# Lynx-MR/orbslam3lib

Measured on AMD Instinct MI355X. Metric: Mfeatures/s extract + Mmatches/s BFMatch, 640x480 stereo 8-level pyr, 1/2/4/8 GPU, higher is better.
Workload: dtype u8; 1 GPU; C2 640x480 stereo, 8 levels x1.2, 2000 feat/frame, FAST 20/7, + per-pair 2000x2000 Hamming kNN2 (left->right, all rows); parallelism=frames sharded across 1 GPU(s), replicas

## Files before the change

### orbslam3lib_amd/csrc/orb_knn2.hip

```cpp
#include <hip/hip_runtime.h>
#include <stdint.h>

#include <algorithm>
#include <type_traits>

#include "orb_kernels.h"

namespace orbgpu {

__device__ inline uint32_t med3_u32(uint32_t a, uint32_t b, uint32_t c) {
    return max(min(a, b), min(max(a, b), c));
}

__device__ inline void knn2_store(uint32_t k1, uint32_t k2, int qi, int32_t* i1, int32_t* d1,
                                  int32_t* i2, int32_t* d2) {
    i1[qi] = k1 == 0xFFFFFFFFu ? -1 : (int32_t)(k1 & 0xFFFF);
    d1[qi] = k1 == 0xFFFFFFFFu ? 0x7fffffff : (int32_t)(k1 >> 16);
    i2[qi] = k2 == 0xFFFFFFFFu ? -1 : (int32_t)(k2 & 0xFFFF);
    d2[qi] = k2 == 0xFFFFFFFFu ? 0x7fffffff : (int32_t)(k2 >> 16);
}

typedef int knn_v8i __attribute__((ext_vector_type(8)));
typedef float knn_v16f __attribute__((ext_vector_type(16)));
constexpr int kKnnWaves = 8;
constexpr int kKnnThreads = 64 * kKnnWaves;
constexpr int kKnnQ = 32 * kKnnWaves;
static_assert(kKnnQ == kKnnQueries, "orb_kernels.h kKnnQueries (grid and arrival counters)");
constexpr int kKnnSeg = 4096;
constexpr int kKnnPitch4 = 144;
__device__ inline uint32_t knn_nib_of(uint32_t ws) {
    uint32_t r;
    asm("v_and_or_b32 %0, %1, %2, %3" : "=v"(r) : "v"(ws), "v"(0x88888888u), "v"(0x22222222u));
    return r;
}
__device__ inline knn_v8i knn4_expand(uint32_t w) {
    knn_v8i v;
    v[0] = (int)knn_nib_of(w << 3);
    v[1] = (int)knn_nib_of(w << 2);
    v[2] = (int)knn_nib_of(w << 1);
    v[3] = (int)knn_nib_of(w);
    v[4] = v[5] = v[6] = v[7] = 0;
    return v;
}
__device__ inline float knn_med3_f32(float a, float b, float c) {
    float r;
    asm("v_med3_f32 %0, %1, %2, %3" : "=v"(r) : "v"(a), "v"(b), "v"(c));
    return r;
}
__device__ inline float knn_max3_f32(float a, float b, float c) {
    float r;
    asm("v_max3_f32 %0, %1, %2, %3" : "=v"(r) : "v"(a), "v"(b), "v"(c));
    return r;
}
__device__ __attribute__((always_inline)) inline void knn2_fp4_block(
    const uint8_t* q, int nq, const uint8_t* t, int nt, int qb, int ts, int te, int32_t* i1, int32_t* d1,
    int32_t* i2, int32_t* d2, uint2* part, uint8_t* lds) {
    const int tid = threadIdx.x, lane = tid & 63, wave = tid >> 6;
    const int r = lane & 31, h = lane >> 5;
    const int qi = qb * kKnnQ + wave * 32 + r;
    knn_v8i qf[4];
    {
        const uint4* qp = reinterpret_cast<const uint4*>(q + (long long)min(qi, max(nq - 1, 0)) * 32);
        const uint4 qa = qp[0], qc = qp[1];
        qf[0] = knn4_expand(h ? qa.y : qa.x);
        qf[1] = knn4_expand(h ? qa.w : qa.z);
        qf[2] = knn4_expand(h ? qc.y : qc.x);
        qf[3] = knn4_expand(h ? qc.w : qc.z);
    }
    uint32_t g1 = 0xFFFFFFFFu, g2 = 0xFFFFFFFFu;
    const int er = tid >> 3, ed = tid & 7;
    const bool expander = tid < 256;
    auto load_packed = [&](int tile) __attribute__((always_inline)) {
        const int row = min(tile * 32 + er, nt - 1);
        return expander ? *reinterpret_cast<const uint32_t*>(t + (long long)row * 32 + 4 * ed) : 0u;
    };
    auto tile_lds = [&](int u) __attribute__((always_inline)) { return lds + ((u - ts) & 1) * (32 * kKnnPitch4); };
    auto store_expanded = [&](int u, uint32_t w) __attribute__((always_inline)) {
        if (expander) {
            const knn_v8i v = knn4_expand(w);
            *reinterpret_cast<uint4*>(tile_lds(u) + er * kKnnPitch4 + 16 * ed) = make_uint4(v[0], v[1], v[2], v[3]);
        }
    };
    uint32_t pk0 = 0, pk1 = 0;
    if (te > ts) {
        store_expanded(ts, load_packed(ts));
        pk1 = load_packed(ts + 1);
    }
    auto rowc = [](int g) { return (g & 3) + 8 * (g >> 2); };
    knn_v16f C0;
#pragma unroll
    for (int g = 0; g < 16; ++g) C0[g] = (float)(4095 - 4 * h - rowc(g));
    const float kNone = -1073741824.0f;
    for (int seg0 = (ts * 32 / kKnnSeg) * kKnnSeg; seg0 < te * 32; seg0 += kKnnSeg) {
        const int tile0 = max(seg0 >> 5, ts), tile1 = min(te, (seg0 + kKnnSeg) >> 5);
        float ka1 = kNone, ka2 = kNone, kb1 = kNone, kb2 = kNone;
        auto select = [&](const knn_v16f& v, bool shift) __attribute__((always_inline)) {
            if (shift) {
                ka1 += 32.f;
                ka2 += 32.f;
                kb1 += 32.f;
                kb2 += 32.f;
            }
#pragma unroll
            for (int g = 0; g < 16; g += 4) {
                const float x0 = v[g], y0 = v[g + 1], x1 = v[g + 2], y1 = v[g + 3];
                ka2 = fmaxf(ka2, knn_med3_f32(ka1, x0, y0));
                ka1 = knn_max3_f32(ka1, x0, y0);
                kb2 = fmaxf(kb2, knn_med3_f32(kb1, x1, y1));
                kb1 = knn_max3_f32(kb1, x1, y1);
            }
        };
        auto body = [&](int ti, auto par, knn_v16f& acc, const knn_v16f& prev) __attribute__((always_inline)) {
            constexpr int PAR = decltype(par)::value;
            uint32_t& pk_use = PAR ? pk0 : pk1;
            uint32_t& pk_load = PAR ? pk1 : pk0;
            __syncthreads();
            pk_load = load_packed(ti + 2);
            const uint8_t* ab = tile_lds(ti) + r * kKnnPitch4 + 16 * h;
#pragma unroll
            for (int s = 0; s < 4; ++s) {
                const uint4 a4 = *reinterpret_cast<const uint4*>(ab + 32 * s);
                const knn_v8i a = {(int)a4.x, (int)a4.y, (int)a4.z, (int)a4.w, 0, 0, 0, 0};
                acc = __builtin_amdgcn_mfma_scale_f32_32x32x64_f8f6f4(a, qf[s], s ? acc : C0, 4, 4, 0, 133, 0, 133);
            }
            if (ti > tile0) select(prev, ti - 1 > tile0);
            if (ti + 1 < te) store_expanded(ti + 1, pk_use);
            if (ti * 32 + 32 > nt) {
#pragma unroll
                for (int g = 0; g < 16; ++g)
                    if (ti * 32 + rowc(g) + 4 * h >= nt) acc[g] = kNone;
            }
        };
        using P0 = std::integral_constant<int, 0>;
        using P1 = std::integral_constant<int, 1>;
        knn_v16f acc0, acc1;
        int ti = tile0;
        for (; ti + 1 < tile1; ti += 2) {
            body(ti, P0{}, acc0, acc1);
            body(ti + 1, P1{}, acc1, acc0);
        }
        if (ti < tile1) {
            body(ti, P0{}, acc0, acc1);
            select(acc0, ti > tile0);
        } else if (tile1 > tile0) {
            select(acc1, tile1 - 1 > tile0);
        }
        const int unbias = 32 * (tile1 - 1 - tile0);
        const int k1 = (int)fmaxf(ka1, kb1) - unbias;
        const int k2 = (int)fmaxf(fminf(ka1, kb1), fmaxf(ka2, kb2)) - unbias;
        auto fold = [&](int k) __attribute__((always_inline)) {
            if (k < -(1 << 24)) return;
            const int tl = 4095 - (k & 4095), dotp = k >> 12;
            const uint32_t key = ((uint32_t)((256 - dotp) >> 1) << 16) | (uint32_t)(32 * tile0 + tl);
            g2 = med3_u32(g1, g2, key);
            g1 = min(g1, key);
        };
        fold(k1);
        fold(k2);
    }
    const uint32_t o1 = __shfl_xor(g1, 32), o2 = __shfl_xor(g2, 32);
    g2 = med3_u32(g1, g2, o1);
    g1 = min(g1, o1);
    g2 = med3_u32(g1, g2, o2);
    g1 = min(g1, o2);
    if (h == 0 && qi < nq) {
        if (part) part[qi] = make_uint2(g1, g2);
        else knn2_store(g1, g2, qi, i1, d1, i2, d2);
    }
}
constexpr int kKnnLdsBytes = 2 * 32 * kKnnPitch4;

__global__ __launch_bounds__(kKnnThreads) void k_knn2_mfma_pairs(MatchArgs m) {
    __shared__ __attribute__((aligned(16))) uint8_t lds[kKnnLdsBytes];
    const int pair = m.pair0 + blockIdx.y;
    const int qimg = 2 * pair, timg = 2 * pair + 1;
    const int qn = m.out_n[qimg], tn = m.out_n[timg];
    const int q0 = m.stereo_only ? m.out_mono[qimg] : 0;
    const int tq0 = m.stereo_only ? m.out_mono[timg] : 0;
    const int nq = qn > q0 ? qn - q0 : 0, nt = tn > tq0 ? tn - tq0 : 0;
    if (blockIdx.x == 0 && threadIdx.x == 0) m.nq[pair] = nq;
    if ((int)blockIdx.x * kKnnQ >= nq) return;
    const uint8_t* q = m.desc + ((long long)qimg * m.out_cap + q0) * 32;
    const uint8_t* t = m.desc + ((long long)timg * m.out_cap + tq0) * 32;
    const long long o = (long long)pair * m.out_cap;
    const int npt = (((nt + 31) >> 5) + 1) >> 1, S = gridDim.z, sp = blockIdx.z;
    const int ts = 2 * (npt * sp / S), te = min((nt + 31) >> 5, 2 * (npt * (sp + 1) / S));
    uint2* part = m.part ? m.part + ((long long)(blockIdx.y * S + sp)) * m.out_cap : nullptr;
    knn2_fp4_block(q, nq, t, nt, blockIdx.x, ts, te, m.idx1 + o, m.dist1 + o, m.idx2 + o, m.dist2 + o, part, lds);
    if (!part || !m.cnt || S == 1) return;
    asm volatile("s_waitcnt vmcnt(0)" ::: "memory");
    __syncthreads();
    int* s_last = reinterpret_cast<int*>(lds);
    if (threadIdx.x == 0) {
        uint32_t* c = m.cnt + blockIdx.y * gridDim.x + blockIdx.x;
        __builtin_amdgcn_fence(__ATOMIC_RELEASE, "agent");
        asm volatile("s_waitcnt vmcnt(0)" ::: "memory");
        const bool last = __hip_atomic_fetch_add(c, 1u, __ATOMIC_RELAXED, __HIP_MEMORY_SCOPE_AGENT) == (uint32_t)(S - 1);
        if (last) {
            __hip_atomic_store(c, 0u, __ATOMIC_RELAXED, __HIP_MEMORY_SCOPE_AGENT);
            __builtin_amdgcn_fence(__ATOMIC_ACQUIRE, "agent");
            asm volatile("s_waitcnt vmcnt(0)" ::: "memory");
        }
        *s_last = last ? 1 : 0;
    }
    __syncthreads();
    if (!*s_last) return;
    const long long pb = (long long)blockIdx.y * S * m.out_cap;
    for (int i = threadIdx.x; i < kKnnQ; i += kKnnThreads) {
        const int qi = blockIdx.x * kKnnQ + i;
        if (qi >= nq) break;
        uint32_t g1 = 0xFFFFFFFFu, g2 = 0xFFFFFFFFu;
        for (int k = 0; k < S; ++k) {
            const uint2 kk = m.part[pb + (long long)k * m.out_cap + qi];
            g2 = med3_u32(g1, g2, kk.x);
            g1 = min(g1, kk.x);
            g2 = med3_u32(g1, g2, kk.y);
            g1 = min(g1, kk.y);
        }
        knn2_store(g1, g2, qi, m.idx1 + o, m.dist1 + o, m.idx2 + o, m.dist2 + o);
    }
}

__global__ __launch_bounds__(256) void k_knn2_merge(MatchArgs m, int nsplit) {
    const int pair = m.pair0 + blockIdx.y;
    const int qimg = 2 * pair, timg = 2 * pair + 1;
    const int qn = m.out_n[qimg], tn = m.out_n[timg];
    const int q0 = m.stereo_only ? m.out_mono[qimg] : 0;
    const int nq = qn > q0 ? qn - q0 : 0;
    (void)tn;
    const int qi = blockIdx.x * 256 + threadIdx.x;
    if (qi >= nq) return;
    uint32_t g1 = 0xFFFFFFFFu, g2 = 0xFFFFFFFFu;
    for (int sp = 0; sp < nsplit; ++sp) {
        const uint2 k = m.part[((long long)(blockIdx.y * nsplit + sp)) * m.out_cap + qi];
        g2 = med3_u32(g1, g2, k.x);
        g1 = min(g1, k.x);
        g2 = med3_u32(g1, g2, k.y);
        g1 = min(g1, k.y);
    }
    const long long o = (long long)pair * m.out_cap;
    knn2_store(g1, g2, qi, m.idx1 + o, m.dist1 + o, m.idx2 + o, m.dist2 + o);
}

__global__ __launch_bounds__(kKnnThreads) void k_knn2_mfma_plain(const uint8_t* q, int nq, const uint8_t* t, int nt,
                                                         int32_t* i1, int32_t* d1, int32_t* i2, int32_t* d2) {
    __shared__ __attribute__((aligned(16))) uint8_t lds[kKnnLdsBytes];
    knn2_fp4_block(q, nq, t, nt, blockIdx.x, 0, (nt + 31) >> 5, i1, d1, i2, d2, nullptr, lds);
}

hipError_t launch_knn2_pairs(const MatchArgs& m, int npairs, hipStream_t s) {
    const int S = m.part ? std::max(1, std::min(kKnnMaxSplit, kKnnSplitSlots / std::max(npairs, 1))) : 1;
    const int qblocks = (m.out_cap + kKnnQ - 1) / kKnnQ;
    if (S > 1) {
        if (npairs * S > kKnnSplitSlots || (m.cnt && (long long)npairs * qblocks > m.cnt_slots))
            return hipErrorInvalidValue;
        hipLaunchKernelGGL(k_knn2_mfma_pairs, dim3(qblocks, npairs, S), dim3(kKnnThreads), 0, s, m);
        if (!m.cnt) hipLaunchKernelGGL(k_knn2_merge, dim3((m.out_cap + 255) / 256, npairs), dim3(256), 0, s, m, S);
        return hipGetLastError();
    }
    MatchArgs m1 = m;
    m1.part = nullptr;
    hipLaunchKernelGGL(k_knn2_mfma_pairs, dim3(qblocks, npairs), dim3(kKnnThreads), 0, s, m1);
    return hipGetLastError();
}
hipError_t launch_knn2_plain(const uint8_t* q, int nq, const uint8_t* t, int nt, int32_t* i1,
                             int32_t* d1, int32_t* i2, int32_t* d2, hipStream_t s) {
    if (nq == 0) return hipSuccess;
    hipLaunchKernelGGL(k_knn2_mfma_plain, dim3((nq + kKnnQ - 1) / kKnnQ), dim3(kKnnThreads), 0, s, q, nq, t, nt, i1,
                       d1, i2, d2);
    return hipGetLastError();
}

}
```

Before: 601.5 Mfeatures/s.

## Deepen kNN2 tile prefetch ring, flatten segment loop, remap blocks across XCDs

Replaces the two-deep packed-descriptor prefetch with a configurable register ring (default depth 3) so global loads of train tiles are issued further ahead of the MFMA work. The segment loop is flattened into a single tile loop, with segment-boundary selection and folding done inside each step, and unrolled by a compile-time integer sequence. The match kernel also remaps block IDs through an XCD-aware mapping so neighbouring blocks share L2 on MI355X. The extra ring registers and larger unroll may raise VGPR pressure and reduce occupancy. Loads are now unconditional for all threads, including those that do not expand.

```diff
diff --git a/orbslam3lib_amd/csrc/orb_knn2.hip b/orbslam3lib_amd/csrc/orb_knn2.hip
--- a/orbslam3lib_amd/csrc/orb_knn2.hip
+++ b/orbslam3lib_amd/csrc/orb_knn2.hip
@@ -3,6 +3,7 @@
 
 #include <algorithm>
 #include <type_traits>
+#include <utility>
 
 #include "orb_kernels.h"
 
@@ -51,6 +52,19 @@
     float r;
     asm("v_max3_f32 %0, %1, %2, %3" : "=v"(r) : "v"(a), "v"(b), "v"(c));
     return r;
+}
+#ifndef KNN_RING
+#define KNN_RING 3
+#endif
+#ifndef KNN_XCD
+#define KNN_XCD 1
+#endif
+constexpr int kKnnRing = KNN_RING;
+static_assert(kKnnRing >= 2, "the step of tile u expands tile u + 1 and loads tile u + kKnnRing");
+template <bool kAll, class F, int... I>
+__device__ __attribute__((always_inline)) inline void knn_steps(F& f, int ti, std::integer_sequence<int, I...>) {
+    if constexpr (kAll) (f(ti + I, std::integral_constant<int, I>{}), ...);
+    else (void)(f(ti + I, std::integral_constant<int, I>{}) && ...);
 }
 __device__ __attribute__((always_inline)) inline void knn2_fp4_block(
     const uint8_t* q, int nq, const uint8_t* t, int nt, int qb, int ts, int te, int32_t* i1, int32_t* d1,
@@ -68,96 +82,92 @@
         qf[3] = knn4_expand(h ? qc.w : qc.z);
     }
     uint32_t g1 = 0xFFFFFFFFu, g2 = 0xFFFFFFFFu;
-    const int er = tid >> 3, ed = tid & 7;
+    const int er = (tid & 255) >> 3, ed = tid & 7;
     const bool expander = tid < 256;
     auto load_packed = [&](int tile) __attribute__((always_inline)) {
         const int row = min(tile * 32 + er, nt - 1);
-        return expander ? *reinterpret_cast<const uint32_t*>(t + (long long)row * 32 + 4 * ed) : 0u;
-    };
-    auto tile_lds = [&](int u) __attribute__((always_inline)) { return lds + ((u - ts) & 1) * (32 * kKnnPitch4); };
-    auto store_expanded = [&](int u, uint32_t w) __attribute__((always_inline)) {
+        return *reinterpret_cast<const uint32_t*>(t + (long long)row * 32 + 4 * ed);
+    };
+    constexpr int kTileBytes = 32 * kKnnPitch4;
+    auto store_expanded = [&](int buf, uint32_t w) __attribute__((always_inline)) {
         if (expander) {
             const knn_v8i v = knn4_expand(w);
-            *reinterpret_cast<uint4*>(tile_lds(u) + er * kKnnPitch4 + 16 * ed) = make_uint4(v[0], v[1], v[2], v[3]);
-        }
-    };
-    uint32_t pk0 = 0, pk1 = 0;
+            *reinterpret_cast<uint4*>(lds + buf * kTileBytes + er * kKnnPitch4 + 16 * ed) = make_uint4(v[0], v[1], v[2], v[3]);
+        }
+    };
+    constexpr int D = kKnnRing, U = D % 2 ? 2 * D : D;
+    uint32_t ring[D];
     if (te > ts) {
-        store_expanded(ts, load_packed(ts));
-        pk1 = load_packed(ts + 1);
+        store_expanded(0, load_packed(ts));
+#pragma unroll
+        for (int j = 1; j < D; ++j) ring[j] = load_packed(ts + j);
     }
     auto rowc = [](int g) { return (g & 3) + 8 * (g >> 2); };
     knn_v16f C0;
 #pragma unroll
     for (int g = 0; g < 16; ++g) C0[g] = (float)(4095 - 4 * h - rowc(g));
     const float kNone = -1073741824.0f;
-    for (int seg0 = (ts * 32 / kKnnSeg) * kKnnSeg; seg0 < te * 32; seg0 += kKnnSeg) {
-        const int tile0 = max(seg0 >> 5, ts), tile1 = min(te, (seg0 + kKnnSeg) >> 5);
-        float ka1 = kNone, ka2 = kNone, kb1 = kNone, kb2 = kNone;
-        auto select = [&](const knn_v16f& v, bool shift) __attribute__((always_inline)) {
-            if (shift) {
-                ka1 += 32.f;
-                ka2 += 32.f;
-                kb1 += 32.f;
-                kb2 += 32.f;
-            }
-#pragma unroll
-            for (int g = 0; g < 16; g += 4) {
-                const float x0 = v[g], y0 = v[g + 1], x1 = v[g + 2], y1 = v[g + 3];
-                ka2 = fmaxf(ka2, knn_med3_f32(ka1, x0, y0));
-                ka1 = knn_max3_f32(ka1, x0, y0);
-                kb2 = fmaxf(kb2, knn_med3_f32(kb1, x1, y1));
-                kb1 = knn_max3_f32(kb1, x1, y1);
-            }
-        };
-        auto body = [&](int ti, auto par, knn_v16f& acc, const knn_v16f& prev) __attribute__((always_inline)) {
-            constexpr int PAR = decltype(par)::value;
-            uint32_t& pk_use = PAR ? pk0 : pk1;
-            uint32_t& pk_load = PAR ? pk1 : pk0;
-            __syncthreads();
-            pk_load = load_packed(ti + 2);
-            const uint8_t* ab = tile_lds(ti) + r * kKnnPitch4 + 16 * h;
-#pragma unroll
-            for (int s = 0; s < 4; ++s) {
-                const uint4 a4 = *reinterpret_cast<const uint4*>(ab + 32 * s);
-                const knn_v8i a = {(int)a4.x, (int)a4.y, (int)a4.z, (int)a4.w, 0, 0, 0, 0};
-                acc = __builtin_amdgcn_mfma_scale_f32_32x32x64_f8f6f4(a, qf[s], s ? acc : C0, 4, 4, 0, 133, 0, 133);
-            }
-            if (ti > tile0) select(prev, ti - 1 > tile0);
-            if (ti + 1 < te) store_expanded(ti + 1, pk_use);
-            if (ti * 32 + 32 > nt) {
-#pragma unroll
-                for (int g = 0; g < 16; ++g)
-                    if (ti * 32 + rowc(g) + 4 * h >= nt) acc[g] = kNone;
-            }
-        };
-        using P0 = std::integral_constant<int, 0>;
-        using P1 = std::integral_constant<int, 1>;
-        knn_v16f acc0, acc1;
-        int ti = tile0;
-        for (; ti + 1 < tile1; ti += 2) {
-            body(ti, P0{}, acc0, acc1);
-            body(ti + 1, P1{}, acc1, acc0);
-        }
-        if (ti < tile1) {
-            body(ti, P0{}, acc0, acc1);
-            select(acc0, ti > tile0);
-        } else if (tile1 > tile0) {
-            select(acc1, tile1 - 1 > tile0);
-        }
-        const int unbias = 32 * (tile1 - 1 - tile0);
-        const int k1 = (int)fmaxf(ka1, kb1) - unbias;
-        const int k2 = (int)fmaxf(fminf(ka1, kb1), fmaxf(ka2, kb2)) - unbias;
-        auto fold = [&](int k) __attribute__((always_inline)) {
-            if (k < -(1 << 24)) return;
-            const int tl = 4095 - (k & 4095), dotp = k >> 12;
-            const uint32_t key = ((uint32_t)((256 - dotp) >> 1) << 16) | (uint32_t)(32 * tile0 + tl);
-            g2 = med3_u32(g1, g2, key);
-            g1 = min(g1, key);
-        };
-        fold(k1);
-        fold(k2);
-    }
+    int tile0 = ts;
+    float ka1 = kNone, ka2 = kNone, kb1 = kNone, kb2 = kNone;
+    auto select = [&](const knn_v16f& v, bool shift) __attribute__((always_inline)) {
+        if (shift) {
+            ka1 += 32.f;
+            ka2 += 32.f;
+            kb1 += 32.f;
+            kb2 += 32.f;
+        }
+#pragma unroll
+        for (int g = 0; g < 16; g += 4) {
+            const float x0 = v[g], y0 = v[g + 1], x1 = v[g + 2], y1 = v[g + 3];
+            ka2 = fmaxf(ka2, knn_med3_f32(ka1, x0, y0));
+            ka1 = knn_max3_f32(ka1, x0, y0);
+            kb2 = fmaxf(kb2, knn_med3_f32(kb1, x1, y1));
+            kb1 = knn_max3_f32(kb1, x1, y1);
+        }
+    };
+    auto fold = [&](int k) __attribute__((always_inline)) {
+        if (k < -(1 << 24)) return;
+        const int tl = 4095 - (k & 4095), dotp = k >> 12;
+        const uint32_t key = ((uint32_t)((256 - dotp) >> 1) << 16) | (uint32_t)(32 * tile0 + tl);
+        g2 = med3_u32(g1, g2, key);
+        g1 = min(g1, key);
+    };
+    knn_v16f acc0, acc1;
+    auto step = [&](int ti, auto ph) __attribute__((always_inline)) -> bool {
+        constexpr int PH = decltype(ph)::value;
+        knn_v16f& acc = PH & 1 ? acc1 : acc0;
+        const knn_v16f& prev = PH & 1 ? acc0 : acc1;
+        __syncthreads();
+        ring[PH % D] = load_packed(ti + D);
+        const uint8_t* ab = lds + (PH & 1) * kTileBytes + r * kKnnPitch4 + 16 * h;
+#pragma unroll
+        for (int s = 0; s < 4; ++s) {
+            const uint4 a4 = *reinterpret_cast<const uint4*>(ab + 32 * s);
+            const knn_v8i a = {(int)a4.x, (int)a4.y, (int)a4.z, (int)a4.w, 0, 0, 0, 0};
+            acc = __builtin_amdgcn_mfma_scale_f32_32x32x64_f8f6f4(a, qf[s], s ? acc : C0, 4, 4, 0, 133, 0, 133);
+        }
+        if (ti > tile0) select(prev, ti - 1 > tile0);
+        if (ti + 1 < te) store_expanded((PH + 1) & 1, ring[(PH + 1) % D]);
+        if (ti * 32 + 32 > nt) {
+#pragma unroll
+            for (int g = 0; g < 16; ++g)
+                if (ti * 32 + rowc(g) + 4 * h >= nt) acc[g] = kNone;
+        }
+        if (ti + 1 == te || ((ti + 1) & (kKnnSeg / 32 - 1)) == 0) {
+            select(acc, ti > tile0);
+            const int unbias = 32 * (ti - tile0);
+            const int k1 = (int)fmaxf(ka1, kb1) - unbias;
+            const int k2 = (int)fmaxf(fminf(ka1, kb1), fmaxf(ka2, kb2)) - unbias;
+            fold(k1);
+            fold(k2);
+            ka1 = ka2 = kb1 = kb2 = kNone;
+            tile0 = ti + 1;
+        }
+        return ti + 1 < te;
+    };
+    int ti = ts;
+    for (; ti + U <= te; ti += U) knn_steps<true>(step, ti, std::make_integer_sequence<int, U>{});
+    if (ti < te) knn_steps<false>(step, ti, std::make_integer_sequence<int, U - 1>{});
     const uint32_t o1 = __shfl_xor(g1, 32), o2 = __shfl_xor(g2, 32);
     g2 = med3_u32(g1, g2, o1);
     g1 = min(g1, o1);
@@ -172,27 +182,34 @@
 
 __global__ __launch_bounds__(kKnnThreads) void k_knn2_mfma_pairs(MatchArgs m) {
     __shared__ __attribute__((aligned(16))) uint8_t lds[kKnnLdsBytes];
-    const int pair = m.pair0 + blockIdx.y;
+#if KNN_XCD
+    const int gx = gridDim.x, gy = gridDim.y;
+    const int wg = xcd_remap(blockIdx.x + gx * (blockIdx.y + gy * blockIdx.z), gx * gy * gridDim.z);
+    const int wrow = wg / gx, bx = wg - wrow * gx, bz = wrow / gy, by = wrow - bz * gy;
+#else
+    const int bx = blockIdx.x, by = blockIdx.y, bz = blockIdx.z;
+#endif
+    const int pair = m.pair0 + by;
     const int qimg = 2 * pair, timg = 2 * pair + 1;
     const int qn = m.out_n[qimg], tn = m.out_n[timg];
     const int q0 = m.stereo_only ? m.out_mono[qimg] : 0;
     const int tq0 = m.stereo_only ? m.out_mono[timg] : 0;
     const int nq = qn > q0 ? qn - q0 : 0, nt = tn > tq0 ? tn - tq0 : 0;
-    if (blockIdx.x == 0 && threadIdx.x == 0) m.nq[pair] = nq;
-    if ((int)blockIdx.x * kKnnQ >= nq) return;
+    if (bx == 0 && bz == 0 && threadIdx.x == 0) m.nq[pair] = nq;
+    if (bx * kKnnQ >= nq) return;
     const uint8_t* q = m.desc + ((long long)qimg * m.out_cap + q0) * 32;
     const uint8_t* t = m.desc + ((long long)timg * m.out_cap + tq0) * 32;
     const long long o = (long long)pair * m.out_cap;
-    const int npt = (((nt + 31) >> 5) + 1) >> 1, S = gridDim.z, sp = blockIdx.z;
+    const int npt = (((nt + 31) >> 5) + 1) >> 1, S = gridDim.z, sp = bz;
     const int ts = 2 * (npt * sp / S), te = min((nt + 31) >> 5, 2 * (npt * (sp + 1) / S));
-    uint2* part = m.part ? m.part + ((long long)(blockIdx.y * S + sp)) * m.out_cap : nullptr;
-    knn2_fp4_block(q, nq, t, nt, blockIdx.x, ts, te, m.idx1 + o, m.dist1 + o, m.idx2 + o, m.dist2 + o, part, lds);
+    uint2* part = m.part ? m.part + ((long long)(by * S + sp)) * m.out_cap : nullptr;
+    knn2_fp4_block(q, nq, t, nt, bx, ts, te, m.idx1 + o, m.dist1 + o, m.idx2 + o, m.dist2 + o, part, lds);
     if (!part || !m.cnt || S == 1) return;
     asm volatile("s_waitcnt vmcnt(0)" ::: "memory");
     __syncthreads();
     int* s_last = reinterpret_cast<int*>(lds);
     if (threadIdx.x == 0) {
-        uint32_t* c = m.cnt + blockIdx.y * gridDim.x + blockIdx.x;
+        uint32_t* c = m.cnt + by * gridDim.x + bx;
         __builtin_amdgcn_fence(__ATOMIC_RELEASE, "agent");
         asm volatile("s_waitcnt vmcnt(0)" ::: "memory");
         const bool last = __hip_atomic_fetch_add(c, 1u, __ATOMIC_RELAXED, __HIP_MEMORY_SCOPE_AGENT) == (uint32_t)(S - 1);
@@ -205,9 +222,9 @@
     }
     __syncthreads();
     if (!*s_last) return;
-    const long long pb = (long long)blockIdx.y * S * m.out_cap;
+    const long long pb = (long long)by * S * m.out_cap;
     for (int i = threadIdx.x; i < kKnnQ; i += kKnnThreads) {
-        const int qi = blockIdx.x * kKnnQ + i;
+        const int qi = bx * kKnnQ + i;
         if (qi >= nq) break;
         uint32_t g1 = 0xFFFFFFFFu, g2 = 0xFFFFFFFFu;
         for (int k = 0; k < S; ++k) {
```

Result: no change. 602.5 Mfeatures/s (median of 5 runs) (+0.2%).
